# apple/ml-4m

Measured on AMD Instinct MI355X. Metric: multimodal tokens/sec (4M-B train step, whole job), higher is better.
Workload: dtype bf16; 1 GPU; 4M-B mod7 (fm_base_12e_12d_swiglu_nobias, 360.8M params, 8 input / 7 target modalities) masked-modeling train step, 224^2 token grids, 128 input + 128 target tokens/sample, AdamW; model=fm_base_12e_12d_swiglu_nobias, per_gpu_batch=256, global_batch=256, seq_len=256, parallelism=dp1

## Files before the change

include/fourm_hip.h:

```cpp
#ifndef FOURM_HIP_H
#define FOURM_HIP_H
#include <stdint.h>

#ifdef __cplusplus
extern "C" {
#endif

#define FM_ABI_VERSION 11
int fm_abi_version(void);
const char* fm_last_error(void);

enum fm_epilogue {
    FM_EPI_BF16 = 0,
    FM_EPI_GELU = 1,
    FM_EPI_RESIDUAL = 2,
    FM_EPI_SWIGLU = 3,
    FM_EPI_F32 = 4,
    FM_EPI_TANH = 5,
    FM_EPI_SWIGLU_BWD = 6,
    FM_EPI_GELU_BWD = 7
};

typedef struct fm_gemm_group {
    const void* W;
// ... 102 lines not shown
    const void* pos;
    const void* mod_emb;
    const void* proj_bias;
    int32_t L;
    int32_t kind, ids_are_i64, mod_id;
    int32_t max_len;
    int32_t shifted;
    int32_t mask_stride, id_stride;
    int32_t patch, channels, grid_w, orig_dim;
    int32_t head_index;
    int32_t pad_;
} fm_mod_desc;

typedef struct fm_select_desc {
    fm_mod_desc mods[FM_MAX_MODS];
    int32_t n_mods, batch, dim, n_keep, n_reg, total_len, is_decoder;
    int32_t raw;
    const void* reg_tokens;
    const void* mask_token;
    void* tokens;
    void* emb;
    void* x0;
    void* out_mask;
    void* out_mod;
    void* slot_mod;
    void* slot_src;
    void* slot_pos;
    void* target_ids;
    void* out_cs;
    void* out_mod_pre;
    void* out_mod_index;
    void* patch_rows;
    void* seqemb_rows;
    int32_t patch_ld, seqemb_ld;
    int32_t rows_f32;
    int32_t pad2_;
} fm_select_desc;
int fm_select_embed(const fm_select_desc* desc, void* stream);

typedef struct fm_embed_bwd_mod {
    void* d_table;
    void* d_pos;
    void* d_mod_emb;
    void* d_proj_bias;
    int32_t kind, has_padding_idx, padding_idx, pad_;
} fm_embed_bwd_mod;
typedef struct fm_embed_bwd_desc {
    fm_embed_bwd_mod mods[FM_MAX_MODS];
    const void* dx;
    const void* slot_mod; const void* slot_src; const void* slot_pos;
    void* d_mask_token;
    void* d_reg_tokens;
    int32_t n_mods, batch, dim, Nt, lddx, is_decoder;
} fm_embed_bwd_desc;
int fm_embed_bwd(const fm_embed_bwd_desc* desc, void* stream);

int fm_dense_decoder_mask(const int32_t* cs, const int16_t* mod, void* out, int B, int M, int causal, int use_cs,
                          int use_sep, void* stream);

enum fm_loss_type { FM_LOSS_MOD = 0, FM_LOSS_TOKEN = 1 };
#define FM_SEG_ROWS 256
int fm_segment_rows(const int32_t* head_of_row, int R, int n_heads, int32_t* seg_start, int32_t* seg_count,
                    int32_t* perm, int32_t* row_to_padded, int32_t* tile_group, int Rp, void* stream);
int fm_gather_rows(const void* src, int ld_src, const int32_t* perm, void* dst, int ld_dst, int Rp, int D, void* stream);
int fm_cross_entropy(void* logits, int ldl, const int32_t* perm, const int32_t* tile_group, const int64_t* target_ids,
                     const int32_t* vocab, const int32_t* seg_start, const int32_t* seg_count, const void* grad_scale,
                     int loss_type, int n_heads, int Rp, int max_vocab, void* row_loss, void* row_lse, void* head_loss,
                     void* total_loss, int write_grad, void* stream);

int fm_swiglu_bwd(const void* da, int ldda, const void* gu, int ldgu, void* dgu, int lddgu, int R, int H, int Hp, void* stream);
int fm_gelu_bwd(const void* dh, int lddh, const void* pre, int ldp, void* dpre, int lddp, int R, int H, int Hp, void* stream);
typedef struct fm_shadow_desc {
    const void* src; void* dst;
    int32_t ld_src, ld_dst, rows, cols, transpose, tile_start;
    const void* col_scale;
    int32_t dst_f32, reserved;
} fm_shadow_desc;
int fm_shadow_refresh(const fm_shadow_desc* descs, int n_descs, int total_tiles, void* stream);
#define FM_FOLD_MAX_JOBS 48
typedef struct fm_fold_grad_job {
    const void* dWp; const void* W; const void* gamma; void* gW; void* ggamma;
    int32_t rows, cols, ld_dwp, reserved;
} fm_fold_grad_job;
int fm_fold_colscale_grad(const fm_fold_grad_job* jobs, int n_jobs, void* stream);

int fm_cast_pad(const void* src, int ld_src, void* dst, int ld_dst, int rows, int cols, void* stream);
int fm_transpose_cast_pad(const void* src, int ld_src, void* dst, int ld_dst, int dst_cols, int rows, int cols, void* stream);
int fm_colsum(const void* dy, int ldy, void* db, int R, int N, void* stream);
int fm_f32_to_bf16(const void* src, void* dst, int64_t n, void* stream);
int fm_bf16_to_f32_scaled(const void* src, void* dst, int64_t n, float scale, void* stream);
int fm_add_bf16_f32(const void* x, const void* delta, void* out, int64_t n, void* stream);
int fm_scale_rows_bf16(void* x, int ld, const void* scale, int rows_per_sample, int R, int N, void* stream);

int fm_vit_patch_rows(const void* pixels, void* rows, int ld, int B, int C, int H, int W, int P, int rows_f32, void* stream);
int fm_vit_emb_rows(const void* pos, const void* mod_emb, void* x, int ldx, int B, int Np, int D, void* stream);
int fm_vit_colsum(const void* dy, int ldy, void* db, int R, int N, void* ws, int64_t ws_bytes, void* stream);

int fm_lora_apply(const void* x, int ldx, const void* down, int64_t down_sr, int64_t down_sk, const void* up, int64_t up_sn, int64_t up_sr,
                  void* y, int ldy, float scale, void* p_out, int R, int K, int N, int r, int x_f32, int y_f32, void* stream);
int fm_lora_grad(const void* a, int lda, const void* b, void* out, int64_t out_sn, int64_t out_sr, float scale, int accumulate,
                 int R, int n, int r, int a_f32, void* stream);

int fm_adamw(void* p, const void* g, void* m, void* v, int64_t n, float lr, float beta1, float beta2, float eps,
             float weight_decay, int64_t step, const void* grad_mult, const void* hyper, void* sumsq, void* stream);
#define FM_ADAMW_CHUNK 8192
typedef struct fm_adamw_job {
// ... 115 lines not shown
```

ml-4m_amd/csrc/select_embed.hip:

```cpp
#include "common.h"
#include "fourm_hip.h"

namespace {

constexpr int MAXPOS = 8192;
constexpr int MAXKEEP = 1024;

struct SelArgs {
    fm_select_desc d;
};

__device__ __forceinline__ long long load_id(const void* ids, int is64, size_t i) {
    return is64 ? ((const long long*)ids)[i] : (long long)((const int*)ids)[i];
}

__device__ __forceinline__ int block_scan_excl(int v, int* wave_tot , int* total) {
    const int lane = threadIdx.x & 63, wave = threadIdx.x >> 6;
    const int inc = wave_scan_incl(v);
    if (lane == 63) wave_tot[wave] = inc;
    __syncthreads();
    int base = 0, tot = 0;
#pragma unroll
    for (int w = 0; w < 4; ++w) {
        const int t = wave_tot[w];
// ... 161 lines not shown
            *(float4*)(emb_o + c * 4) = e;
            if (x0_o) *(float4*)(x0_o + c * 4) = make_float4(t.x + e.x, t.y + e.y, t.z + e.z, t.w + e.w);
        }
        if (d.patch_rows && d.rows_f32) {
            float* pr = (float*)d.patch_rows + orow * d.patch_ld;
            const bool here = (!masked || raw) && md.kind == FM_KIND_PATCH;
            const int ps = md.patch, C = md.channels, gw = md.grid_w;
            const float* img = (const float*)md.ids + (size_t)b * md.id_stride;
            for (int f = lane; f < d.patch_ld; f += 64) {
                float v = 0.f;
                if (here && f < ps * ps * C) {
                    const int gy = j / gw, gx = j % gw, Wd = gw * ps, Hd = (md.L / gw) * ps;
                    const int c = f % C, px = (f / C) % ps, py = f / (C * ps);
                    v = img[((size_t)c * Hd + gy * ps + py) * Wd + gx * ps + px];
                }
                pr[f] = v;
            }
        } else if (d.patch_rows) {
            bf16_t* pr = (bf16_t*)d.patch_rows + orow * d.patch_ld;
            if ((!masked || raw) && md.kind == FM_KIND_PATCH) {
                const int ps = md.patch, C = md.channels, gw = md.grid_w;
                const int gy = j / gw, gx = j % gw;
                const float* img = (const float*)md.ids + (size_t)b * md.id_stride;
                const int Wd = gw * ps, Hd = (md.L / gw) * ps;
                for (int f = lane; f < d.patch_ld; f += 64) {
                    float v = 0.f;
                    if (f < ps * ps * C) {
                        const int c = f % C, px = (f / C) % ps, py = f / (C * ps);
                        v = img[((size_t)c * Hd + gy * ps + py) * Wd + gx * ps + px];
                    }
                    pr[f] = f2bf(v);
                }
            } else {
                for (int f = lane; f < d.patch_ld / 4; f += 64) *(uint2*)(pr + f * 4) = make_uint2(0u, 0u);
            }
        }
        if (d.seqemb_rows && d.rows_f32) {
            float* sr = (float*)d.seqemb_rows + orow * d.seqemb_ld;
            const bool here = (!masked || raw) && md.kind == FM_KIND_SEQ_EMB;
            const float* src = (const float*)md.ids + (size_t)b * md.id_stride + (size_t)j * md.orig_dim;
            for (int f = lane; f < d.seqemb_ld; f += 64) sr[f] = (here && f < md.orig_dim) ? src[f] : 0.f;
        } else if (d.seqemb_rows) {
            bf16_t* sr = (bf16_t*)d.seqemb_rows + orow * d.seqemb_ld;
            if ((!masked || raw) && md.kind == FM_KIND_SEQ_EMB) {
                const float* src = (const float*)md.ids + (size_t)b * md.id_stride + (size_t)j * md.orig_dim;
                for (int f = lane; f < d.seqemb_ld; f += 64) sr[f] = f2bf(f < md.orig_dim ? src[f] : 0.f);
            } else {
                for (int f = lane; f < d.seqemb_ld / 4; f += 64) *(uint2*)(sr + f * 4) = make_uint2(0u, 0u);
            }
        }
    }
}

__global__ __launch_bounds__(256) void embed_bwd_kernel(fm_embed_bwd_desc d) {
    extern __shared__ __attribute__((aligned(16))) char smem[];
    float* acc = (float*)smem;
    const int D = d.dim, nch = D >> 2;
    const int b = blockIdx.x, lane = threadIdx.x & 63, wave = threadIdx.x >> 6;
    const int rows = d.n_mods + 1;
    for (int i = threadIdx.x; i < rows * D; i += 256) acc[i] = 0.f;
    __shared__ int used[FM_MAX_MODS + 1];
    if (threadIdx.x <= FM_MAX_MODS) used[threadIdx.x] = 0;
    __syncthreads();
    constexpr int MAXQ = 8;
    const int parts = 4 * gridDim.y, part = wave + 4 * blockIdx.y;
    const int per = (d.Nt + parts - 1) / parts, s_lo = part * per, s_hi = min(d.Nt, s_lo + per);
    float4 racc[MAXQ];
    int cur = -1;
    bool cur_mask = false;
    auto flush = [&]() {
        if (cur < 0) return;
#pragma unroll
        for (int q = 0; q < MAXQ; ++q) {
            const int c = lane + 64 * q;
            if (c >= nch) break;
            float* a0 = acc + (size_t)cur * D + c * 4;
            atomicAdd(a0, racc[q].x); atomicAdd(a0 + 1, racc[q].y); atomicAdd(a0 + 2, racc[q].z); atomicAdd(a0 + 3, racc[q].w);
            if (cur_mask) {
                float* a1 = acc + (size_t)d.n_mods * D + c * 4;
                atomicAdd(a1, racc[q].x); atomicAdd(a1 + 1, racc[q].y); atomicAdd(a1 + 2, racc[q].z); atomicAdd(a1 + 3, racc[q].w);
            }
        }
    };
    for (int s = s_lo; s < s_hi; ++s) {
        const size_t row = (size_t)b * d.Nt + s;
        const int m = ((const int32_t*)d.slot_mod)[row];
        if (m == -1) continue;
        const float* g = (const float*)d.dx + row * d.lddx;
        if (m == -2) {
            if (d.d_reg_tokens)
                for (int c = lane; c < D; c += 64) unsafeAtomicAdd((float*)d.d_reg_tokens + (size_t)s * D + c, g[c]);
            continue;
        }
        const fm_embed_bwd_mod& md = d.mods[m];
        const int src = ((const int32_t*)d.slot_src)[row];
        const int posrow = ((const int32_t*)d.slot_pos)[row];
        const bool to_mask_token = d.is_decoder && md.kind == FM_KIND_TOK;
        if (m != cur) {
            flush();
            cur = m; cur_mask = to_mask_token;
#pragma unroll
            for (int q = 0; q < MAXQ; ++q) racc[q] = make_float4(0.f, 0.f, 0.f, 0.f);
            if (lane == 0) { used[m] = 1; if (to_mask_token) used[d.n_mods] = 1; }
        }
        float* trow = nullptr;
        if (to_mask_token) {}
        else if ((md.kind == FM_KIND_TOK || md.kind == FM_KIND_SEQ) && md.d_table && !(md.has_padding_idx && src == md.padding_idx))
            trow = (float*)md.d_table + (size_t)src * D;
        else if (md.kind == FM_KIND_SEQ_EMB && md.d_proj_bias) trow = (float*)md.d_proj_bias;
        float* prow = md.d_pos ? (float*)md.d_pos + (size_t)posrow * D : nullptr;
#pragma unroll
        for (int q = 0; q < MAXQ; ++q) {
            const int c = lane + 64 * q;
            if (c >= nch) break;
            const float4 v = *(const float4*)(g + c * 4);
            racc[q].x += v.x; racc[q].y += v.y; racc[q].z += v.z; racc[q].w += v.w;
            if (trow) {
                unsafeAtomicAdd(trow + c * 4, v.x); unsafeAtomicAdd(trow + c * 4 + 1, v.y);
                unsafeAtomicAdd(trow + c * 4 + 2, v.z); unsafeAtomicAdd(trow + c * 4 + 3, v.w);
            }
            if (prow) {
                unsafeAtomicAdd(prow + c * 4, v.x); unsafeAtomicAdd(prow + c * 4 + 1, v.y);
                unsafeAtomicAdd(prow + c * 4 + 2, v.z); unsafeAtomicAdd(prow + c * 4 + 3, v.w);
            }
        }
    }
    flush();
    __syncthreads();
    for (int m = 0; m < d.n_mods; ++m) {
        if (!used[m] || !d.mods[m].d_mod_emb) continue;
        for (int c = threadIdx.x; c < D; c += 256) unsafeAtomicAdd((float*)d.mods[m].d_mod_emb + c, acc[(size_t)m * D + c]);
    }
    if (used[d.n_mods] && d.d_mask_token)
        for (int c = threadIdx.x; c < D; c += 256) unsafeAtomicAdd((float*)d.d_mask_token + c, acc[(size_t)d.n_mods * D + c]);
}

__global__ void dense_decoder_mask_kernel(const int32_t* cs, const int16_t* mod, uint8_t* out, int B, int M, int causal, int use_cs, int use_sep) {
    const size_t i = (size_t)blockIdx.x * 256 + threadIdx.x;
    if (i >= (size_t)B * M * M) return;
    const int k = i % M, q = (i / M) % M, b = i / ((size_t)M * M);
    bool blk = false;
    if (causal) blk = k > q;
    else if (use_cs) blk = k >= cs[(size_t)b * M + q];
    if (use_sep) blk = blk || (mod[(size_t)b * M + q] != mod[(size_t)b * M + k]);
    out[i] = blk ? 1 : 0;
}

}

extern "C" int fm_select_embed(const fm_select_desc* d, void* stream) {
    FM_CHECK_ARG(d && d->tokens && d->emb && d->out_mask && d->out_mod && d->slot_mod && d->slot_src && d->slot_pos, "fm_select_embed: null output");
    FM_CHECK_ARG(d->n_mods > 0 && d->n_mods <= FM_MAX_MODS, "fm_select_embed: n_mods=%d out of range (max %d)", d->n_mods, FM_MAX_MODS);
    FM_CHECK_ARG(d->dim > 0 && d->dim % 4 == 0, "fm_select_embed: dim must be a multiple of 4");
    FM_CHECK_ARG(d->batch > 0 && d->n_keep > 0 && d->n_keep <= (d->raw ? MAXPOS : MAXKEEP), "fm_select_embed: n_keep=%d out of range (max %d)", d->n_keep,
                 d->raw ? MAXPOS : MAXKEEP);
    int total = 0;
    for (int m = 0; m < d->n_mods; ++m) {
        const fm_mod_desc& md = d->mods[m];
        FM_CHECK_ARG(md.L > 0 && md.mask && md.pos && md.mod_emb, "fm_select_embed: modality %d incomplete", m);
        FM_CHECK_ARG(md.kind != FM_KIND_PATCH || (d->patch_rows && md.ids), "fm_select_embed: pixel modality needs patch_rows and pixels");
        FM_CHECK_ARG(md.kind != FM_KIND_SEQ_EMB || (d->seqemb_rows && md.ids), "fm_select_embed: seq_emb modality needs seqemb_rows");
        FM_CHECK_ARG(!((md.kind == FM_KIND_TOK || md.kind == FM_KIND_SEQ) && !(d->is_decoder && md.kind == FM_KIND_TOK)) || md.table, "fm_select_embed: modality %d needs a table", m);
        FM_CHECK_ARG(!d->is_decoder || md.dam || d->raw, "fm_select_embed: decoder modality %d needs decoder_attention_mask", m);
        FM_CHECK_ARG(!(d->raw == 2 && md.kind == FM_KIND_TOK) || md.table, "fm_select_embed: modality %d needs a table", m);
        total += md.L;
    }
    FM_CHECK_ARG(total == d->total_len, "fm_select_embed: total_len=%d but the modalities sum to %d", d->total_len, total);
    FM_CHECK_ARG(total <= MAXPOS, "fm_select_embed: %d concatenated positions exceed %d", total, MAXPOS);
    FM_CHECK_ARG(d->n_keep <= total, "fm_select_embed: n_keep=%d exceeds the %d available positions", d->n_keep, total);
    FM_CHECK_ARG(d->raw >= 0 && d->raw <= 2 && (!d->raw || (d->n_keep == total && d->n_reg == 0)),
                 "fm_select_embed: raw views cover every position (n_keep == total_len) and carry no register tokens");
    FM_CHECK_ARG(!d->is_decoder || (d->target_ids && d->out_cs && d->out_mod_pre && d->out_mod_index && d->mask_token), "fm_select_embed: decoder outputs missing");
    FM_CHECK_ARG(d->n_reg == 0 || d->reg_tokens, "fm_select_embed: register tokens missing");
    FM_CHECK_ARG(d->patch_ld % 4 == 0 && d->seqemb_ld % 4 == 0, "fm_select_embed: side buffers need ld %% 4 == 0");
    const size_t lds = (size_t)total * 9 + (size_t)d->n_keep * 4 + 16;
    static bool once = (hipFuncSetAttribute((const void*)select_embed_kernel, hipFuncAttributeMaxDynamicSharedMemorySize, MAXPOS * 9 + MAXPOS * 4 + 16) == hipSuccess);
    (void)once;
    SelArgs A; A.d = *d;
    const int slices = d->batch >= 2048 ? 1 : d->batch >= 1024 ? 2 : 4;
    hipLaunchKernelGGL(select_embed_kernel, dim3(d->batch, slices), dim3(256), lds, (hipStream_t)stream, A);
    FM_CHECK_LAUNCH("fm_select_embed");
    return 0;
}

extern "C" int fm_embed_bwd(const fm_embed_bwd_desc* d, void* stream) {
    FM_CHECK_ARG(d && d->dx && d->slot_mod && d->slot_src && d->slot_pos, "fm_embed_bwd: null pointer");
    FM_CHECK_ARG(d->n_mods > 0 && d->n_mods <= FM_MAX_MODS && d->dim % 4 == 0 && d->dim <= 2048 && d->lddx % 4 == 0, "fm_embed_bwd: bad shape (dim <= 2048)");
    const size_t lds = (size_t)(d->n_mods + 1) * d->dim * sizeof(float);
    FM_CHECK_ARG(lds <= 150 * 1024, "fm_embed_bwd: %zu bytes of LDS needed", lds);
    static bool once = (hipFuncSetAttribute((const void*)embed_bwd_kernel, hipFuncAttributeMaxDynamicSharedMemorySize, 150 * 1024) == hipSuccess);
    (void)once;
    const int slices = d->batch >= 2048 ? 1 : d->batch >= 1024 ? 2 : 4;
    hipLaunchKernelGGL(embed_bwd_kernel, dim3(d->batch, slices), dim3(256), lds, (hipStream_t)stream, *d);
    FM_CHECK_LAUNCH("fm_embed_bwd");
    return 0;
}

extern "C" int fm_dense_decoder_mask(const int32_t* cs, const int16_t* mod, void* out, int B, int M, int causal, int use_cs, int use_sep, void* stream) {
    FM_CHECK_ARG(out && (causal || !use_cs || cs) && (!use_sep || mod), "fm_dense_decoder_mask: null pointer");
    const size_t n = (size_t)B * M * M;
    hipLaunchKernelGGL(dense_decoder_mask_kernel, dim3((n + 255) / 256), dim3(256), 0, (hipStream_t)stream, cs, mod, (uint8_t*)out, B, M, causal, use_cs, use_sep);
    FM_CHECK_LAUNCH("fm_dense_decoder_mask");
    return 0;
}
```

ml-4m_amd/fourm/hip/_lib.py:

```python
import ctypes as C
import os

FM_MAX_MODS = 24
_LIB_PATH = os.environ.get("FOURM_HIP_LIB") or os.path.join(os.path.dirname(os.path.dirname(os.path.abspath(__file__))), "_lib", "libfourm_hip.so")


class FourmHipUnavailable(ImportError):
    pass


def _load():
    if not os.path.exists(_LIB_PATH):
        raise FourmHipUnavailable(
            f"{_LIB_PATH} is missing - build the gfx950 kernels first: python ml-4m_amd/build_ext.py "
            "(the 4M hot path has no fallback implementation)")
    return C.CDLL(_LIB_PATH)


lib = _load()
lib.fm_last_error.restype = C.c_char_p
lib.fm_abi_version.restype = C.c_int
ABI_VERSION = 11
if lib.fm_abi_version() != ABI_VERSION:
    raise FourmHipUnavailable(f"libfourm_hip.so ABI {lib.fm_abi_version()} != expected {ABI_VERSION}; rebuild")
# ... 58 lines not shown

class ShadowDesc(C.Structure):
    _fields_ = [("src", vp), ("dst", vp), ("ld_src", i32), ("ld_dst", i32), ("rows", i32), ("cols", i32),
                ("transpose", i32), ("tile_start", i32), ("col_scale", vp), ("dst_f32", i32), ("reserved", i32)]


FOLD_MAX_JOBS = 48


class FoldGradJob(C.Structure):
    _fields_ = [("dWp", vp), ("W", vp), ("gamma", vp), ("gW", vp), ("ggamma", vp), ("rows", i32), ("cols", i32), ("ld_dwp", i32), ("reserved", i32)]


class GemmF32Args(C.Structure):
    _fields_ = [("X", vp), ("W", vp), ("W2", vp), ("out", vp), ("out2", vp), ("res", vp), ("bias", vp), ("bias2", vp),
                ("sxm", i64), ("sxk", i64), ("swn", i64), ("swk", i64),
                ("M", i32), ("N", i32), ("K", i32), ("ldo", i32), ("ldo2", i32), ("ldr", i32), ("Hp", i32), ("epilogue", i32),
                ("accumulate", i32), ("max_N", i32), ("seg_rows", i32), ("n_groups", i32),
                ("groups", vp), ("tile_group", vp), ("seg_start", vp), ("seg_count", vp)]


class SpanMaskArgs(C.Structure):
    _fields_ = [("ids", vp), ("len", vp), ("unit", vp), ("noise", vp), ("keep_prob", vp), ("r_choice", vp), ("input_budget", vp), ("target_budget", vp),
                ("sentinel_ids", vp), ("emb", vp), ("emb_out", vp), ("src", vp), ("tensor", vp), ("input_mask", vp), ("target_mask", vp),
                ("decoder_attention_mask", vp), ("tries", vp),
                ("B", i32), ("ld_ids", i32), ("T", i32), ("ld_noise", i32), ("n_sentinels", i32), ("max_tokens", i32), ("vocab_offset", i32), ("pad_id", i32),
                ("emb_rows", i32), ("emb_dim", i32)]


class AdamWJob(C.Structure):
    _fields_ = [("p", vp), ("g", vp), ("m", vp), ("v", vp), ("dst_plain", vp), ("dst_t", vp),
                ("rows", i32), ("cols", i32), ("ld_plain", i32), ("ld_t", i32), ("tile_start", i32), ("pad_", i32)]


class SelectDesc(C.Structure):
    _fields_ = [("mods", ModDesc * FM_MAX_MODS),
                ("n_mods", i32), ("batch", i32), ("dim", i32), ("n_keep", i32), ("n_reg", i32), ("total_len", i32),
                ("is_decoder", i32), ("raw", i32),
                ("reg_tokens", vp), ("mask_token", vp),
                ("tokens", vp), ("emb", vp), ("x0", vp), ("out_mask", vp), ("out_mod", vp), ("slot_mod", vp),
                ("slot_src", vp), ("slot_pos", vp), ("target_ids", vp), ("out_cs", vp), ("out_mod_pre", vp),
                ("out_mod_index", vp), ("patch_rows", vp), ("seqemb_rows", vp), ("patch_ld", i32), ("seqemb_ld", i32),
                ("rows_f32", i32), ("pad2_", i32)]


class EmbedBwdMod(C.Structure):
    _fields_ = [("d_table", vp), ("d_pos", vp), ("d_mod_emb", vp), ("d_proj_bias", vp),
                ("kind", i32), ("has_padding_idx", i32), ("padding_idx", i32), ("pad_", i32)]


class EmbedBwdDesc(C.Structure):
    _fields_ = [("mods", EmbedBwdMod * FM_MAX_MODS), ("dx", vp), ("slot_mod", vp), ("slot_src", vp), ("slot_pos", vp),
                ("d_mask_token", vp), ("d_reg_tokens", vp),
                ("n_mods", i32), ("batch", i32), ("dim", i32), ("Nt", i32), ("lddx", i32), ("is_decoder", i32)]


def _sig(name, *argtypes):
    fn = getattr(lib, name)
    fn.argtypes = list(argtypes)
    fn.restype = C.c_int
    return fn


P = C.POINTER
gemm_nt = _sig("fm_gemm_nt", P(GemmNTArgs), vp)
gemm_tn = _sig("fm_gemm_tn", P(GemmTNArgs), vp)
gemm_tn_multi = _sig("fm_gemm_tn_multi", P(GemmTNJob), C.c_int, vp)
layernorm_fwd = _sig("fm_layernorm_fwd", vp, i32, vp, vp, vp, i32, i32, vp, vp, vp, i32, i32, f32, vp)
layernorm_fwd_res = _sig("fm_layernorm_fwd_res", vp, i32, vp, i32, vp, i32, vp, vp, vp, i32, i32, vp, vp, vp, i32, i32, f32, vp)
layernorm_bwd = _sig("fm_layernorm_bwd", vp, i32, vp, vp, i32, vp, vp, vp, vp, vp, i32, vp, i32, vp, vp, i32, i32, vp)
layernorm_bwd_h = _sig("fm_layernorm_bwd_h", vp, i32, vp, i32, vp, i32, vp, vp, vp, vp, vp, i32, vp, i32, vp, i32, i32, vp)
attn_fwd = _sig("fm_attn_fwd", P(AttnArgs), vp)
attn_bwd = _sig("fm_attn_bwd", P(AttnArgs), vp)
attn_decode = _sig("fm_attn_decode", P(AttnDecodeArgs), vp)
ATTN_DECODE_MAX_NK = 8192
select_embed = _sig("fm_select_embed", P(SelectDesc), vp)
embed_bwd = _sig("fm_embed_bwd", P(EmbedBwdDesc), vp)
dense_decoder_mask = _sig("fm_dense_decoder_mask", vp, vp, vp, i32, i32, i32, i32, i32, vp)
segment_rows = _sig("fm_segment_rows", vp, i32, i32, vp, vp, vp, vp, vp, i32, vp)
gather_rows = _sig("fm_gather_rows", vp, i32, vp, vp, i32, i32, i32, vp)
cross_entropy = _sig("fm_cross_entropy", vp, i32, vp, vp, vp, vp, vp, vp, vp, i32, i32, i32, i32, vp, vp, vp, vp, i32, vp)
swiglu_bwd = _sig("fm_swiglu_bwd", vp, i32, vp, i32, vp, i32, i32, i32, i32, vp)
gelu_bwd = _sig("fm_gelu_bwd", vp, i32, vp, i32, vp, i32, i32, i32, i32, vp)
cast_pad = _sig("fm_cast_pad", vp, i32, vp, i32, i32, i32, vp)
transpose_cast_pad = _sig("fm_transpose_cast_pad", vp, i32, vp, i32, i32, i32, i32, vp)
colsum = _sig("fm_colsum", vp, i32, vp, i32, i32, vp)
shadow_refresh = _sig("fm_shadow_refresh", vp, i32, i32, vp)
fold_colscale_grad = _sig("fm_fold_colscale_grad", vp, i32, vp)
headnorm_fwd = _sig("fm_headnorm_fwd", vp, i32, vp, vp, vp, i32, vp, i32, i32, C.c_float, vp)
headnorm_bwd = _sig("fm_headnorm_bwd", vp, i32, vp, i32, vp, vp, vp, i32, vp, vp, i32, i32, vp)
f32_to_bf16 = _sig("fm_f32_to_bf16", vp, vp, i64, vp)
bf16_to_f32_scaled = _sig("fm_bf16_to_f32_scaled", vp, vp, i64, f32, vp)
add_bf16_f32 = _sig("fm_add_bf16_f32", vp, vp, vp, i64, vp)
lib.fm_set_reserved_cus.argtypes = [C.c_int]
lib.fm_get_reserved_cus.restype = C.c_int
lib.fm_get_reserved_cus.argtypes = []
adamw = _sig("fm_adamw", vp, vp, vp, vp, i64, f32, f32, f32, f32, f32, i64, vp, vp, vp, vp)
adamw_shadow = _sig("fm_adamw_shadow", vp, i32, i32, f32, f32, f32, f32, f32, i64, vp, vp, vp, vp)
sumsq = _sig("fm_sumsq", vp, i64, vp, vp)
clip_coef = _sig("fm_clip_coef", vp, f32, vp, vp, vp)
sample_tokens = _sig("fm_sample_tokens", vp, i32, i32, i32, i32, f32, i32, f32, vp, vp, vp, vp)
maskgit_commit = _sig("fm_maskgit_commit", vp, vp, vp, i32, i32, i32, vp, i32, i32, vp, vp, vp, vp)
gemm_f32 = _sig("fm_gemm_f32", P(GemmF32Args), vp)
attn_f32_fwd = _sig("fm_attn_f32_fwd", P(AttnArgs), vp)
attn_f32_bwd = _sig("fm_attn_f32_bwd", P(AttnArgs), vp)
layernorm_bwd_f32 = _sig("fm_layernorm_bwd_f32", vp, i32, vp, vp, i32, vp, vp, vp, vp, vp, i32, vp, i32, vp, vp, i32, i32, vp)
headnorm_f32_fwd = _sig("fm_headnorm_f32_fwd", vp, i32, vp, vp, vp, i32, vp, i32, i32, C.c_float, vp)
# ... 71 lines not shown
```

ml-4m_amd/fourm/hip/engine.py:

```python
import math
import os
import random
import weakref
from typing import Dict, List, Optional

import torch
import torch.nn as nn

from . import _lib as L
from . import ops

_WEIGHT_EPOCH = 0
FUSE_ACT_BWD = os.environ.get("FOURM_FUSE_ACT_BWD", "0") == "1"
HEADS_DENSE = os.environ.get("FOURM_HEADS_DENSE", "1") == "1"
HEADS_DENSE_MAX = int(os.environ.get("FOURM_HEADS_DENSE_MAX", "8"))
DEFER_RESIDUAL = os.environ.get("FOURM_DEFER_RESIDUAL", "1") == "1"
HOIST_CTX = os.environ.get("FOURM_HOIST_CTX", "1") == "1"
LN_BWD_FROM_H = os.environ.get("FOURM_LN_BWD_FROM_H", "1") == "1"
DP_RESERVE_ALWAYS = os.environ.get("FOURM_DP_RESERVE_ALWAYS", "0") == "1"


def bump_weight_epoch():
    global _WEIGHT_EPOCH
    _WEIGHT_EPOCH += 1
# ... 894 lines not shown
            dqn = ws.get("bwd.dqn", (Rqp, D), bf)
            dkn = ws.get("bwd.dkn", (Rcp, D), bf)
            ops.attn_bwd(sv["xqkn.q"], sv["xqkn.k"], kv[:, D:], sv["o2"], do, dqn, dkn, dkv[:, D:], B, self.H, M, N, self.scale,
                         sv["sm2"], sv["sl2"], zero_attn=getattr(xa, "allow_zero_attn", False), **xa_mask)
            self._qk_norm_bwd(xa, sv, "xqkn", dqn, dkn, sv["q"], kv[:, :D], dq, dkv[:, :D], Rq, Rc)
        else:
            ops.attn_bwd(sv["q"], kv[:, :D], kv[:, D:], sv["o2"], do, dq, dkv[:, :D], dkv[:, D:], B, self.H, M, N, self.scale,
                         sv["sm2"], sv["sl2"], zero_attn=getattr(xa, "allow_zero_attn", False), **xa_mask)
        self._dW(dq, sv["hq"], xa.q, Rq)
        dhq = ws.get("bwd.dh", (Rqp, D), bf)
        ops.gemm_nt(dq, self.wt(xa.q.weight), dhq, M=Rq, N=D, K=D)
        self._lora_bwd(xa.q, dq, sv["hq"], dhq, sv.get("lora.q"), Rq)
        g_bf = ws.get("bwd.dec.gbf2", tuple(g_in.shape), g_in.dtype)
        self._ln_bwd(blk.query_norm, dhq, sv["y1"], sv, "nq", g, g_bf, Rq, dres=g)
        if dp:
            ops.scale_rows_bf16(g_bf, dp[0], M, Rq)
        if hoist is None:
            self._dW(dkv, sv["hc"], xa.kv, Rc)
            dhc = ws.get("bwd.dhc", (Rcp, D), bf)
            ops.gemm_nt(dkv, self.wt(xa.kv.weight), dhc, M=Rc, N=D, K=2 * D)
            self._lora_bwd(xa.kv, dkv, sv["hc"], dhc, sv.get("lora.kv"), Rc)
            self._ln_bwd(blk.context_norm, dhc, ctx, sv, "nc", dctx, dctx_bf, Rc, dres=dctx)
        elif xa.kv.weight.requires_grad or blk.context_norm.weight.requires_grad:
            self._dw_jobs.append((dkv, hoist[1], hoist[2], 2 * D, D, Rc))
        dh = self._self_attn_bwd(blk.self_attn, sv, g_bf, B, M, Rq, Rqp, sa_mask)
        self._flush_dW()
        self._ln_bwd(blk.norm1, dh, sv["y_in"], sv, "n1", g, g_in, Rq, dres=g)

    def _embed_bwd(self, sel, dx, dx_extra, is_dec):
        m = self.model
        embs = m.decoder_embeddings if is_dec else m.encoder_embeddings
        d = L.EmbedBwdDesc()
        for i, n in enumerate(sel["names"]):
            e, md = embs[n], d.mods[i]
            md.kind = e.kind
            if e.kind in (L.KIND_TOK, L.KIND_SEQ) and not (is_dec and e.kind == L.KIND_TOK):
                w = e.token_emb.weight
                md.d_table = self.grad_view(w).data_ptr() if w.requires_grad else None
                pad = e.token_emb.padding_idx
                md.has_padding_idx, md.padding_idx = (1, pad) if pad is not None else (0, 0)
            if isinstance(e.pos_emb, nn.Parameter) and e.pos_emb.requires_grad:
                md.d_pos = self.grad_view(e.pos_emb).data_ptr()
            if e.mod_emb.requires_grad:
                md.d_mod_emb = self.grad_view(e.mod_emb).data_ptr()
            if e.kind == L.KIND_SEQ_EMB and e.emb_proj.bias.requires_grad:
                md.d_proj_bias = self.grad_view(e.emb_proj.bias).data_ptr()
        d.dx, d.lddx = dx.data_ptr(), dx.stride(0)
        d.slot_mod, d.slot_src, d.slot_pos = sel["slot_mod"].data_ptr(), sel["slot_src"].data_ptr(), sel["slot_pos"].data_ptr()
        if is_dec and m.mask_token.requires_grad:
            d.d_mask_token = self.grad_view(m.mask_token).data_ptr()
        if not is_dec and m.num_register_tokens and m.register_tokens.requires_grad:
            d.d_reg_tokens = self.grad_view(m.register_tokens).data_ptr()
        d.n_mods, d.batch, d.dim, d.Nt, d.is_decoder = len(sel["names"]), sel["B"], self.D, sel["Nt"], 1 if is_dec else 0
        with ops._prof("embed_bwd"):
            L.check(L.embed_bwd(ops.C.byref(d), ops._stream()))
        if dx_extra is not None:
            d2 = L.EmbedBwdDesc()
            ops.C.memmove(ops.C.byref(d2), ops.C.byref(d), ops.C.sizeof(d))
            for i in range(d.n_mods):
                d2.mods[i].d_table = None
                d2.mods[i].d_proj_bias = None
            d2.d_reg_tokens = None
            d2.dx, d2.lddx = dx_extra.data_ptr(), dx_extra.stride(0)
            with ops._prof("embed_bwd"):
                L.check(L.embed_bwd(ops.C.byref(d2), ops._stream()))

    def train_backward(self, grad_scale: torch.Tensor):
        c = self._ctx
        if c is None:
            raise RuntimeError("train_backward without a preceding training forward")
        self._ctx, self._dw_jobs = None, None
        if self.reducer is not None:
            self.reducer.begin()
            if getattr(self.reducer, "reserved_cus", 0):
                L.lib.fm_set_reserved_cus(int(self.reducer.reserved_cus))
        m, ws = self.model, self.ws
        enc, dec, st, hs = c["enc"], c["dec"], c["st"], c["hs"]
        B, N, Mt, D = enc["B"], enc["Nt"], dec["Nt"], self.D
        bf, f32 = self.adt, torch.float32
        Rq, Rc = B * Mt, B * N
        Rqp, Rcp = st["y_final"].shape[0], st["x_final"].shape[0]
        ops.cross_entropy(hs["logits"], hs["perm"], hs["tile_group"], dec["target_ids"].view(-1), hs["vocab_t"], hs["seg_start"],
                          hs["seg_count"], hs["n"], hs["maxV"], hs["row_loss"], hs["row_lse"], hs["head_loss"], hs["total"],
                          loss_type=hs["loss_type"], grad_scale=grad_scale, write_grad=True)
        dyp = ws.get("bwd.dyp", (hs["Rp"], D), bf)
        ops.gemm_nt_grouped(hs["logits"], hs["g_bwd"], hs["tile_group"], dyp, D, max_K=ru(hs["maxV"], 64))
        heads = [m.decoder_embeddings[h] for h in hs["heads"]]
        if any(h.to_logits.weight.requires_grad for h in heads):
            outs = [self.grad_view(h.to_logits.weight) if h.to_logits.weight.requires_grad else None for h in heads]
            key = tuple(o.data_ptr() if o is not None else 0 for o in outs)
            cache = getattr(self, "_head_tn_groups", None)
            if cache is None or cache[0] != key:
                cache = self._head_tn_groups = (key, ops.make_groups(
                    [dict(out=o, N=(v if o is not None else 0)) for o, v in zip(outs, hs["vocabs"])], self.device))
            tn = cache[1]
            ops.gemm_tn_grouped(hs["logits"], hs["yp"], tn, hs["seg_start"], hs["seg_count"], hs["n"], hs["maxV"], hs["Rp"], D)
        g = ws.get("bwd.g_dec", (Rqp, D), f32)
        g_bf = ws.get("bwd.g_dec_bf", (Rqp, D), bf)
        self._ln_bwd(m.decoder_norm, dyp, st["y_final"], hs["sv"], "dn", g, g_bf, Rq, dres=None, dy_row_map=hs["r2p"])
        self._stage("heads")
        dctx = ws.get("bwd.dctx", (Rcp, D), f32)
        dctx_bf = ws.get("bwd.dctx_bf", (Rcp, D), bf)
        Ld = len(m.decoder)
        ctx_hat = st.get("ctx_hat")
        if ctx_hat is None:
            with ops._prof("fills"):
                dctx.zero_()
        else:
            dkv_all = ws.get("bwd.dkv_all", (Rcp, Ld * 2 * D), bf)
            dwp = ws.get("bwd.dwp", (Ld, 2 * D, D), f32)
            with ops._prof("fills"):
                dwp.zero_()
        for i in reversed(range(Ld)):
            sv = st["dec_layers"][i]
            if "ckpt_in" in sv:
                y_in, dp, sv = sv["ckpt_in"], sv["dp"], {}
                self.decoder_block_fwd(m.decoder[i], y_in, st["ctx"], B, Mt, N, st["smask"], st["emask"], sv, "ckpt", out_name="ckpt.out", dp=dp,
                                       ctx_hat=ctx_hat)
# ... 42 lines not shown
```

Before: 1.174 million tokens/s.

## Fuse dual-gradient embed backward and batch slot loads with ballot-driven row processing

The embedding backward kernel now takes an optional second gradient buffer (dx2), so the decoder's extra gradient is summed in the same launch rather than in a second kernel that rereads slot metadata. Slot metadata is read 64 rows at a time, and live rows are compacted with a ballot. Gradient rows are loaded four at a time to raise memory-level parallelism, and columns are processed in templated chunks. A variant without atomics is selected when no table, position or bias gradients are needed. This trades more template instantiations and register pressure for less launch overhead and fewer redundant reads. The embed backward is a small part of the whole train step.

```diff
diff --git a/include/fourm_hip.h b/include/fourm_hip.h
--- a/include/fourm_hip.h
+++ b/include/fourm_hip.h
@@ -178,6 +178,8 @@
     void* d_mask_token;
     void* d_reg_tokens;
     int32_t n_mods, batch, dim, Nt, lddx, is_decoder;
+    const void* dx2;
+    int32_t lddx2, pad2_;
 } fm_embed_bwd_desc;
 int fm_embed_bwd(const fm_embed_bwd_desc* desc, void* stream);
 
diff --git a/ml-4m_amd/csrc/select_embed.hip b/ml-4m_amd/csrc/select_embed.hip
--- a/ml-4m_amd/csrc/select_embed.hip
+++ b/ml-4m_amd/csrc/select_embed.hip
@@ -237,80 +237,162 @@
     }
 }
 
+constexpr int EB_SLOTS = 4;
+
+template <int VEC, int KB, bool ATOM, bool DX2>
 __global__ __launch_bounds__(256) void embed_bwd_kernel(fm_embed_bwd_desc d) {
     extern __shared__ __attribute__((aligned(16))) char smem[];
     float* acc = (float*)smem;
-    const int D = d.dim, nch = D >> 2;
+    const int D = d.dim;
     const int b = blockIdx.x, lane = threadIdx.x & 63, wave = threadIdx.x >> 6;
     const int rows = d.n_mods + 1;
     for (int i = threadIdx.x; i < rows * D; i += 256) acc[i] = 0.f;
     __shared__ int used[FM_MAX_MODS + 1];
     if (threadIdx.x <= FM_MAX_MODS) used[threadIdx.x] = 0;
     __syncthreads();
-    constexpr int MAXQ = 8;
+    constexpr int CW = 64 * VEC * KB;
     const int parts = 4 * gridDim.y, part = wave + 4 * blockIdx.y;
     const int per = (d.Nt + parts - 1) / parts, s_lo = part * per, s_hi = min(d.Nt, s_lo + per);
-    float4 racc[MAXQ];
+    const float* dx = (const float*)d.dx;
+    const float* dx2 = (const float*)d.dx2;
+    const bool reg_dst = ATOM && d.d_reg_tokens != nullptr;
+    float racc[KB][VEC];
     int cur = -1;
     bool cur_mask = false;
-    auto flush = [&]() {
-        if (cur < 0) return;
-#pragma unroll
-        for (int q = 0; q < MAXQ; ++q) {
-            const int c = lane + 64 * q;
-            if (c >= nch) break;
-            float* a0 = acc + (size_t)cur * D + c * 4;
-            atomicAdd(a0, racc[q].x); atomicAdd(a0 + 1, racc[q].y); atomicAdd(a0 + 2, racc[q].z); atomicAdd(a0 + 3, racc[q].w);
-            if (cur_mask) {
-                float* a1 = acc + (size_t)d.n_mods * D + c * 4;
-                atomicAdd(a1, racc[q].x); atomicAdd(a1 + 1, racc[q].y); atomicAdd(a1 + 2, racc[q].z); atomicAdd(a1 + 3, racc[q].w);
-            }
-        }
-    };
-    for (int s = s_lo; s < s_hi; ++s) {
-        const size_t row = (size_t)b * d.Nt + s;
-        const int m = ((const int32_t*)d.slot_mod)[row];
-        if (m == -1) continue;
-        const float* g = (const float*)d.dx + row * d.lddx;
-        if (m == -2) {
-            if (d.d_reg_tokens)
-                for (int c = lane; c < D; c += 64) unsafeAtomicAdd((float*)d.d_reg_tokens + (size_t)s * D + c, g[c]);
-            continue;
-        }
-        const fm_embed_bwd_mod& md = d.mods[m];
-        const int src = ((const int32_t*)d.slot_src)[row];
-        const int posrow = ((const int32_t*)d.slot_pos)[row];
-        const bool to_mask_token = d.is_decoder && md.kind == FM_KIND_TOK;
-        if (m != cur) {
+    for (int s0 = s_lo; s0 < s_hi; s0 += 64) {
+        const int cnt = min(64, s_hi - s0);
+        int my_m = -1, my_src = 0, my_pos = 0;
+        if (lane < cnt) {
+            const size_t row = (size_t)b * d.Nt + s0 + lane;
+            my_m = ((const int32_t*)d.slot_mod)[row];
+            if (ATOM) { my_src = ((const int32_t*)d.slot_src)[row]; my_pos = ((const int32_t*)d.slot_pos)[row]; }
+        }
+        const unsigned long long live0 = __ballot(my_m >= 0 || (my_m == -2 && reg_dst));
+        for (int cb = 0; cb < D; cb += CW) {
+            int col[KB];
+            bool okc[KB];
+#pragma unroll
+            for (int k = 0; k < KB; ++k) {
+                const int c = cb + (k * 64 + lane) * VEC;
+                okc[k] = c < D;
+                col[k] = okc[k] ? c : D - VEC;
+            }
+            auto flush = [&]() {
+                if (cur < 0) return;
+#pragma unroll
+                for (int k = 0; k < KB; ++k) {
+                    if (!okc[k]) continue;
+                    float* a0 = acc + (size_t)cur * D + col[k];
+                    float* a1 = acc + (size_t)d.n_mods * D + col[k];
+#pragma unroll
+                    for (int j = 0; j < VEC; ++j) {
+                        atomicAdd(a0 + j, racc[k][j]);
+                        if (cur_mask) atomicAdd(a1 + j, racc[k][j]);
+                    }
+                }
+                cur = -1;
+            };
+            unsigned long long live = live0, last = 1;
+            while (live) {
+                int idx[EB_SLOTS];
+                bool oks[EB_SLOTS];
+                float v[EB_SLOTS][KB][VEC], w[DX2 ? EB_SLOTS : 1][KB][VEC];
+#pragma unroll
+                for (int i = 0; i < EB_SLOTS; ++i) {
+                    oks[i] = live != 0;
+                    idx[i] = __ffsll(oks[i] ? live : last) - 1;
+                    last = 1ull << idx[i];
+                    live &= live - 1;
+                    const size_t row = (size_t)b * d.Nt + s0 + idx[i];
+                    const float* g = dx + row * d.lddx;
+                    const float* g2 = DX2 ? dx2 + row * d.lddx2 : nullptr;
+#pragma unroll
+                    for (int k = 0; k < KB; ++k) {
+                        if constexpr (VEC == 4) {
+                            const float4 t = *(const float4*)(g + col[k]);
+                            v[i][k][0] = t.x; v[i][k][1] = t.y; v[i][k][2] = t.z; v[i][k][3] = t.w;
+                            if constexpr (DX2) {
+                                const float4 u = *(const float4*)(g2 + col[k]);
+                                w[i][k][0] = u.x; w[i][k][1] = u.y; w[i][k][2] = u.z; w[i][k][3] = u.w;
+                            }
+                        } else {
+#pragma unroll
+                            for (int j = 0; j < VEC; ++j) {
+                                v[i][k][j] = g[col[k] + j];
+                                if constexpr (DX2) w[i][k][j] = g2[col[k] + j];
+                            }
+                        }
+                    }
+                }
+#pragma unroll
+                for (int i = 0; i < EB_SLOTS; ++i) {
+                    if (!oks[i]) continue;
+                    const int m = __builtin_amdgcn_readfirstlane(__shfl(my_m, idx[i], 64));
+                    const int s = s0 + idx[i];
+                    if (m == -2) {
+                        if (ATOM) {
+                            float* rrow = (float*)d.d_reg_tokens + (size_t)s * D;
+#pragma unroll
+                            for (int k = 0; k < KB; ++k) {
+                                if (!okc[k]) continue;
+#pragma unroll
+                                for (int j = 0; j < VEC; ++j) unsafeAtomicAdd(rrow + col[k] + j, v[i][k][j]);
+                            }
+                        }
+                        continue;
+                    }
+                    const fm_embed_bwd_mod& md = d.mods[m];
+                    const bool to_mask_token = d.is_decoder && md.kind == FM_KIND_TOK;
+                    if (m != cur) {
+                        flush();
+                        cur = m; cur_mask = to_mask_token;
+#pragma unroll
+                        for (int k = 0; k < KB; ++k)
+#pragma unroll
+                            for (int j = 0; j < VEC; ++j) racc[k][j] = 0.f;
+                        if (lane == 0) { used[m] = 1; if (to_mask_token) used[d.n_mods] = 1; }
+                    }
+#pragma unroll
+                    for (int k = 0; k < KB; ++k)
+#pragma unroll
+                        for (int j = 0; j < VEC; ++j) {
+                            racc[k][j] += v[i][k][j];
+                            if constexpr (DX2) racc[k][j] += w[i][k][j];
+                        }
+                    if (ATOM) {
+                        const int src = __builtin_amdgcn_readfirstlane(__shfl(my_src, idx[i], 64));
+                        const int posrow = __builtin_amdgcn_readfirstlane(__shfl(my_pos, idx[i], 64));
+                        float* trow = nullptr;
+                        if (to_mask_token) {}
+                        else if ((md.kind == FM_KIND_TOK || md.kind == FM_KIND_SEQ) && md.d_table && !(md.has_padding_idx && src == md.padding_idx))
+                            trow = (float*)md.d_table + (size_t)src * D;
+                        else if (md.kind == FM_KIND_SEQ_EMB && md.d_proj_bias) trow = (float*)md.d_proj_bias;
+                        float* prow = md.d_pos ? (float*)md.d_pos + (size_t)posrow * D : nullptr;
+                        if (trow) {
+#pragma unroll
+                            for (int k = 0; k < KB; ++k) {
+                                if (!okc[k]) continue;
+#pragma unroll
+                                for (int j = 0; j < VEC; ++j) unsafeAtomicAdd(trow + col[k] + j, v[i][k][j]);
+                            }
+                        }
+                        if (prow) {
+#pragma unroll
+                            for (int k = 0; k < KB; ++k) {
+                                if (!okc[k]) continue;
+#pragma unroll
+                                for (int j = 0; j < VEC; ++j) {
+                                    unsafeAtomicAdd(prow + col[k] + j, v[i][k][j]);
+                                    if constexpr (DX2) unsafeAtomicAdd(prow + col[k] + j, w[i][k][j]);
+                                }
+                            }
+                        }
+                    }
+                }
+            }
             flush();
-            cur = m; cur_mask = to_mask_token;
-#pragma unroll
-            for (int q = 0; q < MAXQ; ++q) racc[q] = make_float4(0.f, 0.f, 0.f, 0.f);
-            if (lane == 0) { used[m] = 1; if (to_mask_token) used[d.n_mods] = 1; }
-        }
-        float* trow = nullptr;
-        if (to_mask_token) {}
-        else if ((md.kind == FM_KIND_TOK || md.kind == FM_KIND_SEQ) && md.d_table && !(md.has_padding_idx && src == md.padding_idx))
-            trow = (float*)md.d_table + (size_t)src * D;
-        else if (md.kind == FM_KIND_SEQ_EMB && md.d_proj_bias) trow = (float*)md.d_proj_bias;
-        float* prow = md.d_pos ? (float*)md.d_pos + (size_t)posrow * D : nullptr;
-#pragma unroll
-        for (int q = 0; q < MAXQ; ++q) {
-            const int c = lane + 64 * q;
-            if (c >= nch) break;
-            const float4 v = *(const float4*)(g + c * 4);
-            racc[q].x += v.x; racc[q].y += v.y; racc[q].z += v.z; racc[q].w += v.w;
-            if (trow) {
-                unsafeAtomicAdd(trow + c * 4, v.x); unsafeAtomicAdd(trow + c * 4 + 1, v.y);
-                unsafeAtomicAdd(trow + c * 4 + 2, v.z); unsafeAtomicAdd(trow + c * 4 + 3, v.w);
-            }
-            if (prow) {
-                unsafeAtomicAdd(prow + c * 4, v.x); unsafeAtomicAdd(prow + c * 4 + 1, v.y);
-                unsafeAtomicAdd(prow + c * 4 + 2, v.z); unsafeAtomicAdd(prow + c * 4 + 3, v.w);
-            }
-        }
-    }
-    flush();
+        }
+    }
     __syncthreads();
     for (int m = 0; m < d.n_mods; ++m) {
         if (!used[m] || !d.mods[m].d_mod_emb) continue;
@@ -318,6 +400,28 @@
     }
     if (used[d.n_mods] && d.d_mask_token)
         for (int c = threadIdx.x; c < D; c += 256) unsafeAtomicAdd((float*)d.d_mask_token + c, acc[(size_t)d.n_mods * D + c]);
+}
+
+template <int VEC, int KB, bool ATOM, bool DX2>
+void embed_bwd_launch(const fm_embed_bwd_desc* d, int slices, size_t lds, hipStream_t stream) {
+    auto kern = embed_bwd_kernel<VEC, KB, ATOM, DX2>;
+    static bool once = (hipFuncSetAttribute((const void*)kern, hipFuncAttributeMaxDynamicSharedMemorySize, 150 * 1024) == hipSuccess);
+    (void)once;
+    hipLaunchKernelGGL(kern, dim3(d->batch, slices), dim3(256), lds, stream, *d);
+}
+
+template <bool ATOM, bool DX2>
+void embed_bwd_dispatch(const fm_embed_bwd_desc* d, int slices, size_t lds, hipStream_t stream) {
+    const int wc = d->dim <= 256 ? 0 : (d->dim <= 768 || d->dim % 768 == 0) ? 1 : 2;
+    if (ATOM) {
+        if (wc == 0) embed_bwd_launch<1, 4, ATOM, DX2>(d, slices, lds, stream);
+        else if (wc == 1) embed_bwd_launch<1, 12, ATOM, DX2>(d, slices, lds, stream);
+        else embed_bwd_launch<1, 16, ATOM, DX2>(d, slices, lds, stream);
+    } else {
+        if (wc == 0) embed_bwd_launch<4, 1, ATOM, DX2>(d, slices, lds, stream);
+        else if (wc == 1) embed_bwd_launch<4, 3, ATOM, DX2>(d, slices, lds, stream);
+        else embed_bwd_launch<4, 4, ATOM, DX2>(d, slices, lds, stream);
+    }
 }
 
 __global__ void dense_decoder_mask_kernel(const int32_t* cs, const int16_t* mod, uint8_t* out, int B, int M, int causal, int use_cs, int use_sep) {
@@ -370,13 +474,18 @@
 
 extern "C" int fm_embed_bwd(const fm_embed_bwd_desc* d, void* stream) {
     FM_CHECK_ARG(d && d->dx && d->slot_mod && d->slot_src && d->slot_pos, "fm_embed_bwd: null pointer");
-    FM_CHECK_ARG(d->n_mods > 0 && d->n_mods <= FM_MAX_MODS && d->dim % 4 == 0 && d->dim <= 2048 && d->lddx % 4 == 0, "fm_embed_bwd: bad shape (dim <= 2048)");
+    FM_CHECK_ARG(d->n_mods > 0 && d->n_mods <= FM_MAX_MODS && d->dim > 0 && d->dim % 4 == 0 && d->dim <= 2048 && d->lddx % 4 == 0 && d->lddx >= d->dim,
+                 "fm_embed_bwd: bad shape (dim <= 2048)");
+    FM_CHECK_ARG(!d->dx2 || (d->lddx2 % 4 == 0 && d->lddx2 >= d->dim), "fm_embed_bwd: bad lddx2");
+    FM_CHECK_ARG(((((uintptr_t)d->dx) | ((uintptr_t)d->dx2)) & 15) == 0, "fm_embed_bwd: gradients must be 16-byte aligned");
+    FM_CHECK_ARG(d->batch > 0 && d->Nt > 0, "fm_embed_bwd: empty launch");
     const size_t lds = (size_t)(d->n_mods + 1) * d->dim * sizeof(float);
     FM_CHECK_ARG(lds <= 150 * 1024, "fm_embed_bwd: %zu bytes of LDS needed", lds);
-    static bool once = (hipFuncSetAttribute((const void*)embed_bwd_kernel, hipFuncAttributeMaxDynamicSharedMemorySize, 150 * 1024) == hipSuccess);
-    (void)once;
     const int slices = d->batch >= 2048 ? 1 : d->batch >= 1024 ? 2 : 4;
-    hipLaunchKernelGGL(embed_bwd_kernel, dim3(d->batch, slices), dim3(256), lds, (hipStream_t)stream, *d);
+    bool atom = d->d_reg_tokens != nullptr;
+    for (int m = 0; m < d->n_mods; ++m) atom = atom || d->mods[m].d_table || d->mods[m].d_pos || d->mods[m].d_proj_bias;
+    if (atom) { if (d->dx2) embed_bwd_dispatch<true, true>(d, slices, lds, (hipStream_t)stream); else embed_bwd_dispatch<true, false>(d, slices, lds, (hipStream_t)stream); }
+    else { if (d->dx2) embed_bwd_dispatch<false, true>(d, slices, lds, (hipStream_t)stream); else embed_bwd_dispatch<false, false>(d, slices, lds, (hipStream_t)stream); }
     FM_CHECK_LAUNCH("fm_embed_bwd");
     return 0;
 }
diff --git a/ml-4m_amd/fourm/hip/_lib.py b/ml-4m_amd/fourm/hip/_lib.py
--- a/ml-4m_amd/fourm/hip/_lib.py
+++ b/ml-4m_amd/fourm/hip/_lib.py
@@ -134,7 +134,8 @@
 class EmbedBwdDesc(C.Structure):
     _fields_ = [("mods", EmbedBwdMod * FM_MAX_MODS), ("dx", vp), ("slot_mod", vp), ("slot_src", vp), ("slot_pos", vp),
                 ("d_mask_token", vp), ("d_reg_tokens", vp),
-                ("n_mods", i32), ("batch", i32), ("dim", i32), ("Nt", i32), ("lddx", i32), ("is_decoder", i32)]
+                ("n_mods", i32), ("batch", i32), ("dim", i32), ("Nt", i32), ("lddx", i32), ("is_decoder", i32),
+                ("dx2", vp), ("lddx2", i32), ("pad2_", i32)]
 
 
 def _sig(name, *argtypes):
diff --git a/ml-4m_amd/fourm/hip/engine.py b/ml-4m_amd/fourm/hip/engine.py
--- a/ml-4m_amd/fourm/hip/engine.py
+++ b/ml-4m_amd/fourm/hip/engine.py
@@ -970,18 +970,10 @@
         if not is_dec and m.num_register_tokens and m.register_tokens.requires_grad:
             d.d_reg_tokens = self.grad_view(m.register_tokens).data_ptr()
         d.n_mods, d.batch, d.dim, d.Nt, d.is_decoder = len(sel["names"]), sel["B"], self.D, sel["Nt"], 1 if is_dec else 0
+        if dx_extra is not None:
+            d.dx2, d.lddx2 = dx_extra.data_ptr(), dx_extra.stride(0)
         with ops._prof("embed_bwd"):
             L.check(L.embed_bwd(ops.C.byref(d), ops._stream()))
-        if dx_extra is not None:
-            d2 = L.EmbedBwdDesc()
-            ops.C.memmove(ops.C.byref(d2), ops.C.byref(d), ops.C.sizeof(d))
-            for i in range(d.n_mods):
-                d2.mods[i].d_table = None
-                d2.mods[i].d_proj_bias = None
-            d2.d_reg_tokens = None
-            d2.dx, d2.lddx = dx_extra.data_ptr(), dx_extra.stride(0)
-            with ops._prof("embed_bwd"):
-                L.check(L.embed_bwd(ops.C.byref(d2), ops._stream()))
 
     def train_backward(self, grad_scale: torch.Tensor):
         c = self._ctx
```

After: 1.181 million tokens/s (median of 6 runs). Within noise of the previous version (+0.6%).
